# 331658260/Drone-YOLO

Hardware: AMD Instinct MI355X
Metric: images/sec @640x640 Drone-YOLO-s (higher is better)
Workload: dtype fp16; 1 GPU; Drone-YOLO-s (yolov8s-p2-repvgg.yaml, nc=10) inference 640x640: layout+forward+decode+NMS, inputs resident in HBM; fp16 storage / fp32 accumulate (BASELINE config 2 names bf16: bf16 storage fails the IoU >= 0.999 bar - 0.995 - so the headline runs the 16-bit format that meets it; same MFMA rate, same bytes); batch_per_gpu=256, global_batch=256, parallelism=batch-split x1, no collective, hipgraph=True, streams=2, max_det=300

## Files before the change

drone-yolo_amd/csrc/conv3x3_hreg.hip:

```cpp
#include "common_hip.h"
#include "conv_args.h"

namespace DY_NS {


struct HregArgs {
  const void* x;
  const void* w;
  const float* bias;
  const void* res;
  void* y;
  int N, H, W, Cin, ldx, Cout, ldy, ldres, act;
  int tilesX, tilesY, tilesN, nSpatial;
  unsigned x_bytes, y_bytes, r_bytes;
  double* stats;
  const float* bnb_mean;
  const float* bnb_rstd;
  const float* bnb_gamma;
  const float* bnb_beta;
  int bnb_act;
  int dbg;
};

#ifdef DYOLO_ABLATE
#define HR_DBG(bit) (p.dbg & (bit))
#else
#define HR_DBG(bit) 0
#endif

constexpr int kHrTH = 8, kHrTW = 16, kHrHH = 10, kHrHW = 24;
constexpr int kHrStage = 16 * 1024;
constexpr int kHrStages = 3;

template <typename T, int NCH, bool RES, bool STATS = false, bool BNB = false, int BW = 3>
__global__ __launch_bounds__(256, NCH <= 2 ? (BNB ? BW : 3) : 2) void conv3x3_hreg_kernel(const HregArgs p) {
  static_assert(!(BNB && (RES || STATS)), "BNB: its own mode");
  constexpr bool SLOTS = STATS || BNB, RLOAD = RES || BNB;
  constexpr int EPC = Elem<T>::EPC;
  __shared__ __attribute__((aligned(1024))) unsigned char smem[kHrStages * kHrStage];
  __shared__ f32x4 bnc[BNB ? 64 : 1];
  const int tid = threadIdx.x, lane = tid & 63, wave = tid >> 6;
  const int lq = lane >> 4, lr = lane & 15;
  const __amdgpu_buffer_rsrc_t yrs = __builtin_amdgcn_make_buffer_rsrc(p.y, 0, p.y_bytes, 0x00020000);
  const __amdgpu_buffer_rsrc_t rrs = __builtin_amdgcn_make_buffer_rsrc(const_cast<void*>(p.res ? p.res : p.y), 0, p.res ? p.r_bytes : 0u, 0x00020000);

  const int G = (int)gridDim.x;
  const int logical = ((int)blockIdx.x & 7) * (G >> 3) + ((int)blockIdx.x >> 3);
  const int nt = logical % p.tilesN;
  const int sb = logical / p.tilesN, Gs = G / p.tilesN;
  const int myTiles = sb < p.nSpatial ? (p.nSpatial - sb + Gs - 1) / Gs : 0;
  if constexpr (SLOTS) {
    if (blockIdx.x == 0)
      for (int i = tid; i < 2 * p.Cout; i += 256) p.stats[i] = 0.0;
    if (myTiles <= 0 && tid < 128) {
      const int co = nt * 64 + (tid & 63);
      if (co < p.Cout) p.stats[(size_t)(1 + sb) * 2 * p.Cout + (tid >> 6) * p.Cout + co] = 0.0;
    }
  }
  if (myTiles <= 0) return;
  const int nItems = myTiles * NCH;

  u32x4 wreg[NCH][9];
  {
    const u32x4* wg = reinterpret_cast<const u32x4*>(p.w) + (size_t)nt * NCH * 9 * 4 * 64;
#pragma unroll
    for (int c = 0; c < NCH; ++c)
#pragma unroll
      for (int t = 0; t < 9; ++t) wreg[c][t] = wg[((c * 9 + t) * 4 + wave) * 64 + lane];
  }
  const f32x4 bias4 = *reinterpret_cast<const f32x4*>(p.bias + nt * 64 + wave * 16 + lq * 4);

  constexpr int NDMA = 4;
  constexpr unsigned kOob = 0xfffffff0u;
  const unsigned pre = (unsigned)((p.W + 1) * p.ldx) * 2u;
  const __amdgpu_buffer_rsrc_t xrs = __builtin_amdgcn_make_buffer_rsrc(const_cast<char*>(reinterpret_cast<const char*>(p.x)) - pre, 0, p.x_bytes + pre, 0x00020000);
  unsigned rel[NDMA];
  int hyx[NDMA];
#pragma unroll
  for (int k = 0; k < NDMA; ++k) {
    const int s = (k * 4 + wave) * 64 + lane;
    const int pix = s >> 2, part = s & 3;
    const int hy = pix / kHrHW, hx = pix - hy * kHrHW;
    const bool dead = hx >= kHrTW + 2 || hy >= kHrHH;
    rel[k] = dead ? kOob : (unsigned)((hy * p.W + hx) * p.ldx + (part ^ ((hx >> 1) & 3)) * EPC) * 2u;
    hyx[k] = hy | (hx << 8);
  }
  unsigned voff[NDMA];
  unsigned l_base = 0;
  int l_tile = sb, l_chunk = 0, l_item = 0;
  auto setup_tile = [&](int tile) {
    const int tx = tile % p.tilesX;
    const int r = tile / p.tilesX;
    const int ty = r % p.tilesY, n = r / p.tilesY;
    const int y0 = ty * kHrTH, x0 = tx * kHrTW;
    l_base = (unsigned)(((n * p.H + y0) * p.W + x0) * p.ldx) * 2u;
    const bool interior = y0 > 0 && y0 + kHrTH + 1 <= p.H && x0 > 0 && x0 + kHrTW + 1 <= p.W;
    if (interior) {
#pragma unroll
      for (int k = 0; k < NDMA; ++k) voff[k] = rel[k];
    } else {
#pragma unroll
      for (int k = 0; k < NDMA; ++k) {
        const int gy = y0 - 1 + (hyx[k] & 255), gx = x0 - 1 + (hyx[k] >> 8);
        voff[k] = ((unsigned)gy < (unsigned)p.H && (unsigned)gx < (unsigned)p.W) ? rel[k] : kOob;
      }
    }
  };
  auto issue_dma = [&](int stage) {
    unsigned char* sa = smem + stage * kHrStage;
    const bool live = l_item < nItems && !(HR_DBG(4) && l_item >= 2);
    if (live) {
      const unsigned soff = l_base + (unsigned)l_chunk * (4u * EPC * (unsigned)sizeof(T));
#pragma unroll
      for (int k = 0; k < NDMA; ++k)
        __builtin_amdgcn_raw_ptr_buffer_load_lds(xrs, (__attribute__((address_space(3))) void*)(sa + (k * 4 + wave) * 1024), 16, (int)voff[k], (int)soff, 0, 0);
      ++l_item;
      if (++l_chunk == NCH) {
        l_chunk = 0;
        l_tile += Gs;
        if (l_item < nItems) setup_tile(l_tile);
      }
    } else {
#pragma unroll
      for (int k = 0; k < NDMA; ++k)
        __builtin_amdgcn_raw_ptr_buffer_load_lds(xrs, (__attribute__((address_space(3))) void*)(sa + (k * 4 + wave) * 1024), 16, (int)kOob, 0, 0, 0);
    }
  };

  int lane_base[3];
#pragma unroll
  for (int q = 0; q < 3; ++q) lane_base[q] = (lr + q) * 64 + ((lq ^ (((lr + q) >> 1) & 3)) * 16);

  f32x4 acc[kHrTH];
#pragma unroll
  for (int o = 0; o < kHrTH; ++o) acc[o] = bias4;

  auto compute = [&](int stg, int c) {
    const unsigned char* sa = smem + stg * kHrStage;
#pragma unroll
    for (int iy = 0; iy < kHrHH; ++iy) {
      u32x4 a[3];
#pragma unroll
      for (int q = 0; q < 3; ++q) a[q] = *reinterpret_cast<const u32x4*>(sa + lane_base[q] + (HR_DBG(8) ? 0 : iy * (kHrHW * 64)));
#pragma unroll
      for (int r = 0; r < 3; ++r) {
        const int o = iy - r;
        if (o >= 0 && o < kHrTH) {
#pragma unroll
          for (int q = 0; q < 3; ++q) {
            if (HR_DBG(2)) asm volatile("" ::"v"(a[q]));
            else acc[o] = Elem<T>::mma(wreg[c][r * 3 + q], a[q], acc[o]);
          }
        }
      }
    }
  };

  typedef __attribute__((ext_vector_type(4))) T t4;
  u32x4 rl[kHrTH / 2];
  auto load_residual = [&](int tile) {
    const int tx = tile % p.tilesX;
    const int r = tile / p.tilesX;
    const int ty = r % p.tilesY, n = r / p.tilesY;
    const int xx = tx * kHrTW + lr;
    const int co16 = nt * 64 + wave * 16 + (lq >> 1) * 8;
#pragma unroll
    for (int o = 0; o < kHrTH; o += 2) {
      const int yy = ty * kHrTH + o + (lq & 1);
      const bool ok = yy < p.H && xx < p.W;
      const unsigned off = ok ? (unsigned)((((size_t)(n * p.H + yy) * p.W + xx) * (size_t)p.ldres + co16) * sizeof(T)) : 0xfffffff0u;
      rl[o / 2] = __builtin_amdgcn_raw_buffer_load_b128(rrs, off, 0, 0);
    }
  };
  unsigned lane_out[kHrTH / 2];
  {
    const int co16 = nt * 64 + wave * 16 + (lq >> 1) * 8;
#pragma unroll
    for (int o = 0; o < kHrTH; o += 2) lane_out[o / 2] = (unsigned)(((o + (lq & 1)) * p.W + lr) * p.ldy + co16) * (unsigned)sizeof(T);
  }
  float st_sum[4] = {0.f, 0.f, 0.f, 0.f}, st_sq[4] = {0.f, 0.f, 0.f, 0.f};
  if constexpr (BNB) {
    if (tid < 64) {
      const int co = nt * 64 + tid;
      const float mu = p.bnb_mean[co], rs = p.bnb_rstd[co], gr = p.bnb_gamma[co] * rs;
      bnc[tid] = f32x4{rs, -mu * rs, gr, p.bnb_beta[co] - gr * mu};
    }
    asm volatile("s_waitcnt lgkmcnt(0)" ::: "memory");
  }
  auto epilogue = [&](int tile) {
    const int tx = tile % p.tilesX;
    const int r = tile / p.tilesX;
    const int ty = r % p.tilesY, n = r / p.tilesY;
    const int y0 = ty * kHrTH, x0 = tx * kHrTW;
    const unsigned out_base = (unsigned)(((n * p.H + y0) * p.W + x0) * p.ldy) * (unsigned)sizeof(T);
    const bool whole = y0 + kHrTH <= p.H && x0 + kHrTW <= p.W;
    u32x2 pk[kHrTH];
#pragma unroll
    for (int o = 0; o < kHrTH; ++o) {
      float v[4] = {acc[o][0], acc[o][1], acc[o][2], acc[o][3]};
      if (p.act == DY_ACT_SILU) {
#pragma unroll
        for (int e = 0; e < 4; ++e) v[e] = silu_f32(v[e]);
      }
      if constexpr (RES) {
        const auto sx = __builtin_amdgcn_permlane16_swap(rl[o / 2][0], rl[o / 2][2], false, false);
        const auto sy = __builtin_amdgcn_permlane16_swap(rl[o / 2][1], rl[o / 2][3], false, false);
        const t4 rr = __builtin_bit_cast(t4, u32x2{sx[o & 1], sy[o & 1]});
#pragma unroll
        for (int e = 0; e < 4; ++e) v[e] += Elem<T>::to_f32(rr[e]);
      }
      t4 ov;
#pragma unroll
      for (int e = 0; e < 4; ++e) ov[e] = Elem<T>::from_f32(v[e]);
      if constexpr (STATS) {
        if (whole || (y0 + o < p.H && x0 + lr < p.W)) {
#pragma unroll
          for (int e = 0; e < 4; ++e) {
            const float f = Elem<T>::to_f32(ov[e]);
            st_sum[e] += f, st_sq[e] += f * f;
          }
        }
      }
      if constexpr (BNB) {
        const auto sx = __builtin_amdgcn_permlane16_swap(rl[o / 2][0], rl[o / 2][2], false, false);
        const auto sy = __builtin_amdgcn_permlane16_swap(rl[o / 2][1], rl[o / 2][3], false, false);
        const t4 zz = __builtin_bit_cast(t4, u32x2{sx[o & 1], sy[o & 1]});
        if (whole || (y0 + o < p.H && x0 + lr < p.W)) {
#pragma unroll
          for (int e = 0; e < 4; ++e) {
            const f32x4 k = bnc[wave * 16 + lq * 4 + e];
            const float zf = Elem<T>::to_f32(zz[e]);
            const float xh = zf * k[0] + k[1];
            float du = Elem<T>::to_f32(ov[e]);
            if (p.bnb_act == DY_ACT_SILU) {
              const float u = zf * k[2] + k[3];
              const float sg = __builtin_amdgcn_rcpf(1.0f + __builtin_amdgcn_exp2f(u * -1.4426950408889634f));
              du *= sg * (1.0f + u * (1.0f - sg));
            }
            st_sum[e] += du, st_sq[e] += du * xh;
          }
        }
      }
      pk[o] = __builtin_bit_cast(u32x2, ov);
      acc[o] = bias4;
    }
#pragma unroll
    for (int o = 0; o < kHrTH; o += 2) {
      const auto sx = __builtin_amdgcn_permlane16_swap(pk[o][0], pk[o + 1][0], false, false);
      const auto sy = __builtin_amdgcn_permlane16_swap(pk[o][1], pk[o + 1][1], false, false);
      unsigned off = lane_out[o / 2];
      if (!whole) off = (y0 + o + (lq & 1) < p.H && x0 + lr < p.W) ? off : kOob;
      __builtin_amdgcn_raw_buffer_store_b128(u32x4{sx[0], sy[0], sx[1], sy[1]}, yrs, HR_DBG(1) ? kOob : off, (int)out_base, 0);
    }
  };

  setup_tile(l_tile);
  issue_dma(0);
  issue_dma(1 % kHrStages);
  asm volatile("s_waitcnt vmcnt(0)" ::: "memory");
  __builtin_amdgcn_s_barrier();
  int c_tile = sb;
  int stage = 0;
  for (int it = 0; it < nItems; it += NCH) {
#pragma unroll
    for (int c = 0; c < NCH; ++c) {
      if constexpr (RLOAD) {
        if (c == NCH - 1) load_residual(c_tile);
      }
      issue_dma(stage + 2 >= kHrStages ? stage + 2 - kHrStages : stage + 2);
      compute(stage, c);
      if (c == NCH - 1) {
        epilogue(c_tile);
        c_tile += Gs;
      }
      asm volatile("s_waitcnt vmcnt(0)" ::: "memory");
      __builtin_amdgcn_s_barrier();
      stage = stage + 1 == kHrStages ? 0 : stage + 1;
    }
  }
  if constexpr (SLOTS) {
#pragma unroll
    for (int e = 0; e < 4; ++e) {
      float a = st_sum[e], b = st_sq[e];
#pragma unroll
      for (int m = 1; m < 16; m <<= 1) a += __shfl_xor(a, m, 64), b += __shfl_xor(b, m, 64);
      const int co = nt * 64 + wave * 16 + lq * 4 + e;
      if (lr == 0 && co < p.Cout) {
        double* slot = p.stats + (size_t)(1 + sb) * 2 * p.Cout;
        slot[co] = (double)a, slot[p.Cout + co] = (double)b;
      }
    }
  }
}

constexpr int kH2TH = 4, kH2TW = 16, kH2HH = 9, kH2Pitch = 40, kH2PlaneB = 24;
constexpr int kH2Stage = 24 * 1024;

template <typename T, int NCH, bool STATS = false>
__global__ __launch_bounds__(256, 2) void conv3x3_hreg_s2_kernel(const HregArgs p) {
  constexpr int EPC = Elem<T>::EPC;
  __shared__ __attribute__((aligned(1024))) unsigned char smem[kHrStages * kH2Stage];
  const int tid = threadIdx.x, lane = tid & 63, wave = tid >> 6;
  const int lq = lane >> 4, lr = lane & 15;
  const __amdgpu_buffer_rsrc_t yrs = __builtin_amdgcn_make_buffer_rsrc(p.y, 0, p.y_bytes, 0x00020000);
  const int Ho = (p.H - 1) / 2 + 1, Wo = (p.W - 1) / 2 + 1;

  const int G = (int)gridDim.x;
  const int logical = ((int)blockIdx.x & 7) * (G >> 3) + ((int)blockIdx.x >> 3);
  const int nt = logical % p.tilesN;
  const int sb = logical / p.tilesN, Gs = G / p.tilesN;
  const int myTiles = sb < p.nSpatial ? (p.nSpatial - sb + Gs - 1) / Gs : 0;
  if constexpr (STATS) {
    if (blockIdx.x == 0)
      for (int i = tid; i < 2 * p.Cout; i += 256) p.stats[i] = 0.0;
    if (myTiles <= 0 && tid < 128) {
      const int co = nt * 64 + (tid & 63);
      if (co < p.Cout) p.stats[(size_t)(1 + sb) * 2 * p.Cout + (tid >> 6) * p.Cout + co] = 0.0;
    }
  }
  if (myTiles <= 0) return;
  const int nItems = myTiles * NCH;

  u32x4 wreg[NCH][9];
  {
    const u32x4* wg = reinterpret_cast<const u32x4*>(p.w) + (size_t)nt * NCH * 9 * 4 * 64;
#pragma unroll
    for (int c = 0; c < NCH; ++c)
#pragma unroll
      for (int t = 0; t < 9; ++t) wreg[c][t] = wg[((c * 9 + t) * 4 + wave) * 64 + lane];
  }
  const f32x4 bias4 = *reinterpret_cast<const f32x4*>(p.bias + nt * 64 + wave * 16 + lq * 4);

  constexpr int NDMA = 6;
  constexpr unsigned kOob = 0xfffffff0u;
  const unsigned pre = (unsigned)((p.W + 1) * p.ldx) * 2u;
  const __amdgpu_buffer_rsrc_t xrs = __builtin_amdgcn_make_buffer_rsrc(const_cast<char*>(reinterpret_cast<const char*>(p.x)) - pre, 0, p.x_bytes + pre, 0x00020000);
  unsigned rel[NDMA];
  int hyx[NDMA];
#pragma unroll
  for (int k = 0; k < NDMA; ++k) {
    const int s = (k * 4 + wave) * 64 + lane;
    const int slot = s >> 2, part = s & 3;
    const int hy = slot / kH2Pitch, c = slot - hy * kH2Pitch;
    const bool planeB = c >= kH2PlaneB;
    const int ci = planeB ? c - kH2PlaneB : c;
    const int hx = planeB ? 2 * ci + 1 : 2 * ci;
    const bool dead = hy >= kH2HH || hx > 2 * kH2TW;
    rel[k] = dead ? kOob : (unsigned)((hy * p.W + hx) * p.ldx + (part ^ ((ci >> 1) & 3)) * EPC) * 2u;
    hyx[k] = hy | (hx << 8);
  }
  unsigned voff[NDMA];
  unsigned l_base = 0;
  int l_tile = sb, l_chunk = 0, l_item = 0;
  auto setup_tile = [&](int tile) {
    const int tx = tile % p.tilesX;
    const int r = tile / p.tilesX;
    const int ty = r % p.tilesY, n = r / p.tilesY;
    const int y0 = 2 * ty * kH2TH, x0 = 2 * tx * kH2TW;
    l_base = (unsigned)(((n * p.H + y0) * p.W + x0) * p.ldx) * 2u;
    const bool interior = y0 > 0 && y0 - 1 + kH2HH <= p.H && x0 > 0 && x0 + 2 * kH2TW <= p.W;
    if (interior) {
#pragma unroll
      for (int k = 0; k < NDMA; ++k) voff[k] = rel[k];
    } else {
#pragma unroll
      for (int k = 0; k < NDMA; ++k) {
        const int gy = y0 - 1 + (hyx[k] & 255), gx = x0 - 1 + (hyx[k] >> 8);
        voff[k] = ((unsigned)gy < (unsigned)p.H && (unsigned)gx < (unsigned)p.W) ? rel[k] : kOob;
      }
    }
  };
  auto issue_dma = [&](int stage) {
    unsigned char* sa = smem + stage * kH2Stage;
    const bool live = l_item < nItems;
    if (live) {
      const unsigned soff = l_base + (unsigned)l_chunk * (4u * EPC * (unsigned)sizeof(T));
#pragma unroll
      for (int k = 0; k < NDMA; ++k)
        __builtin_amdgcn_raw_ptr_buffer_load_lds(xrs, (__attribute__((address_space(3))) void*)(sa + (k * 4 + wave) * 1024), 16, (int)voff[k], (int)soff, 0, 0);
      ++l_item;
      if (++l_chunk == NCH) {
        l_chunk = 0;
        l_tile += Gs;
        if (l_item < nItems) setup_tile(l_tile);
      }
    } else {
#pragma unroll
      for (int k = 0; k < NDMA; ++k)
        __builtin_amdgcn_raw_ptr_buffer_load_lds(xrs, (__attribute__((address_space(3))) void*)(sa + (k * 4 + wave) * 1024), 16, (int)kOob, 0, 0, 0);
    }
  };

  int lane_base[3];
  lane_base[0] = lr * 64 + ((lq ^ ((lr >> 1) & 3)) * 16);
  lane_base[1] = (kH2PlaneB + lr) * 64 + ((lq ^ ((lr >> 1) & 3)) * 16);
  lane_base[2] = (lr + 1) * 64 + ((lq ^ (((lr + 1) >> 1) & 3)) * 16);

  f32x4 acc[kH2TH];
#pragma unroll
  for (int o = 0; o < kH2TH; ++o) acc[o] = bias4;

  auto compute = [&](int stg, int c) {
    const unsigned char* sa = smem + stg * kH2Stage;
#pragma unroll
    for (int iy = 0; iy < kH2HH; ++iy) {
      u32x4 a[3];
#pragma unroll
      for (int q = 0; q < 3; ++q) a[q] = *reinterpret_cast<const u32x4*>(sa + lane_base[q] + iy * (kH2Pitch * 64));
#pragma unroll
      for (int r = 0; r < 3; ++r) {
        if ((iy - r) % 2 == 0) {
          const int o = (iy - r) / 2;
          if (iy - r >= 0 && o < kH2TH) {
#pragma unroll
            for (int q = 0; q < 3; ++q) acc[o] = Elem<T>::mma(wreg[c][r * 3 + q], a[q], acc[o]);
          }
        }
      }
    }
  };

  typedef __attribute__((ext_vector_type(4))) T t4;
  unsigned lane_out[kH2TH / 2];
  {
    const int co16 = nt * 64 + wave * 16 + (lq >> 1) * 8;
#pragma unroll
    for (int o = 0; o < kH2TH; o += 2) lane_out[o / 2] = (unsigned)(((o + (lq & 1)) * Wo + lr) * p.ldy + co16) * (unsigned)sizeof(T);
  }
  float st_sum[4] = {0.f, 0.f, 0.f, 0.f}, st_sq[4] = {0.f, 0.f, 0.f, 0.f};
  auto epilogue = [&](int tile) {
    const int tx = tile % p.tilesX;
    const int r = tile / p.tilesX;
    const int ty = r % p.tilesY, n = r / p.tilesY;
    const int y0 = ty * kH2TH, x0 = tx * kH2TW;
    const unsigned out_base = (unsigned)(((n * Ho + y0) * Wo + x0) * p.ldy) * (unsigned)sizeof(T);
    const bool whole = y0 + kH2TH <= Ho && x0 + kH2TW <= Wo;
    u32x2 pk[kH2TH];
#pragma unroll
    for (int o = 0; o < kH2TH; ++o) {
      float v[4] = {acc[o][0], acc[o][1], acc[o][2], acc[o][3]};
      if (p.act == DY_ACT_SILU) {
#pragma unroll
        for (int e = 0; e < 4; ++e) v[e] = silu_f32(v[e]);
      }
      t4 ov;
#pragma unroll
      for (int e = 0; e < 4; ++e) ov[e] = Elem<T>::from_f32(v[e]);
      pk[o] = __builtin_bit_cast(u32x2, ov);
      if constexpr (STATS) {
        if (whole || (y0 + o < Ho && x0 + lr < Wo)) {
#pragma unroll
          for (int e = 0; e < 4; ++e) {
            const float f = Elem<T>::to_f32(ov[e]);
            st_sum[e] += f, st_sq[e] += f * f;
          }
        }
      }
      acc[o] = bias4;
    }
#pragma unroll
    for (int o = 0; o < kH2TH; o += 2) {
      const auto sx = __builtin_amdgcn_permlane16_swap(pk[o][0], pk[o + 1][0], false, false);
      const auto sy = __builtin_amdgcn_permlane16_swap(pk[o][1], pk[o + 1][1], false, false);
      unsigned off = lane_out[o / 2];
      if (!whole) off = (y0 + o + (lq & 1) < Ho && x0 + lr < Wo) ? off : kOob;
      __builtin_amdgcn_raw_buffer_store_b128(u32x4{sx[0], sy[0], sx[1], sy[1]}, yrs, off, (int)out_base, 0);
    }
  };

  setup_tile(l_tile);
  issue_dma(0);
  issue_dma(1);
  asm volatile("s_waitcnt vmcnt(0)" ::: "memory");
  __builtin_amdgcn_s_barrier();
  int c_tile = sb;
  int stage = 0;
  for (int it = 0; it < nItems; it += NCH) {
#pragma unroll
    for (int c = 0; c < NCH; ++c) {
      issue_dma(stage + 2 >= kHrStages ? stage + 2 - kHrStages : stage + 2);
      compute(stage, c);
      if (c == NCH - 1) {
        epilogue(c_tile);
        c_tile += Gs;
      }
      asm volatile("s_waitcnt vmcnt(0)" ::: "memory");
      __builtin_amdgcn_s_barrier();
      stage = stage + 1 == kHrStages ? 0 : stage + 1;
    }
  }
  if constexpr (STATS) {
#pragma unroll
    for (int e = 0; e < 4; ++e) {
      float a = st_sum[e], b = st_sq[e];
#pragma unroll
      for (int m = 1; m < 16; m <<= 1) a += __shfl_xor(a, m, 64), b += __shfl_xor(b, m, 64);
      const int co = nt * 64 + wave * 16 + lq * 4 + e;
      if (lr == 0 && co < p.Cout) {
        double* slot = p.stats + (size_t)(1 + sb) * 2 * p.Cout;
        slot[co] = (double)a, slot[p.Cout + co] = (double)b;
      }
    }
  }
}

[[maybe_unused]] constexpr int kBnbWgs = 2;
template <typename T>
static int launch_hreg(const HregArgs& a, hipStream_t st) {
  HregArgs p = a;
  const int nch = p.Cin / 32;
  int grid = 256 * (nch <= 2 ? 3 : 2);
  const long long nwork = (long long)p.nSpatial * p.tilesN;
  if (nwork < grid) grid = (int)nwork;
  const int q = 8 * p.tilesN;
  grid = (grid + q - 1) / q * q;
  const bool res = p.res != nullptr;
#ifndef DYOLO_L2E_BUILD
  if (p.bnb_mean) {
    static const int bw = dy_ablate("DYOLO_BNB_WGS") ? dy_ablate("DYOLO_BNB_WGS") : kBnbWgs;
    if (nch == 2 && bw == 2) {
      int g2 = 256 * 2;
      if (nwork < g2) g2 = (int)nwork;
      grid = (g2 + q - 1) / q * q;
      hipLaunchKernelGGL((conv3x3_hreg_kernel<T, 2, false, false, true, 2>), dim3((unsigned)grid), dim3(256), 0, st, p);
    } else if (nch == 2) {
      hipLaunchKernelGGL((conv3x3_hreg_kernel<T, 2, false, false, true, 3>), dim3((unsigned)grid), dim3(256), 0, st, p);
    } else {
      hipLaunchKernelGGL((conv3x3_hreg_kernel<T, 4, false, false, true>), dim3((unsigned)grid), dim3(256), 0, st, p);
    }
    note_stats(grid / p.tilesN);
    return check_launch("conv3x3_hreg_kernel<bnb>");
  }
#endif
  if (p.stats) {
    if (nch == 1) hipLaunchKernelGGL((conv3x3_hreg_kernel<T, 1, false, true>), dim3((unsigned)grid), dim3(256), 0, st, p);
    else if (nch == 2) hipLaunchKernelGGL((conv3x3_hreg_kernel<T, 2, false, true>), dim3((unsigned)grid), dim3(256), 0, st, p);
    else hipLaunchKernelGGL((conv3x3_hreg_kernel<T, 4, false, true>), dim3((unsigned)grid), dim3(256), 0, st, p);
    note_stats(grid / p.tilesN);
    return check_launch("conv3x3_hreg_kernel");
  }
  if (nch == 1) {
    if (res) hipLaunchKernelGGL((conv3x3_hreg_kernel<T, 1, true>), dim3((unsigned)grid), dim3(256), 0, st, p);
    else hipLaunchKernelGGL((conv3x3_hreg_kernel<T, 1, false>), dim3((unsigned)grid), dim3(256), 0, st, p);
  } else if (nch == 2) {
    if (res) hipLaunchKernelGGL((conv3x3_hreg_kernel<T, 2, true>), dim3((unsigned)grid), dim3(256), 0, st, p);
    else hipLaunchKernelGGL((conv3x3_hreg_kernel<T, 2, false>), dim3((unsigned)grid), dim3(256), 0, st, p);
  } else {
    hipLaunchKernelGGL((conv3x3_hreg_kernel<T, 4, false>), dim3((unsigned)grid), dim3(256), 0, st, p);
  }
  return check_launch("conv3x3_hreg_kernel");
}

template <typename T>
static int launch_hreg_s2(const HregArgs& a, hipStream_t st) {
  HregArgs p = a;
  int grid = 256 * 2;
  const long long nwork = (long long)p.nSpatial * p.tilesN;
  if (nwork < grid) grid = (int)nwork;
  const int q = 8 * p.tilesN;
  grid = (grid + q - 1) / q * q;
#ifndef DYOLO_L2E_BUILD
  if (p.stats) {
    hipLaunchKernelGGL((conv3x3_hreg_s2_kernel<T, 2, true>), dim3((unsigned)grid), dim3(256), 0, st, p);
    note_stats(grid / p.tilesN);
    return check_launch("conv3x3_hreg_s2_kernel");
  }
#endif
  hipLaunchKernelGGL((conv3x3_hreg_s2_kernel<T, 2>), dim3((unsigned)grid), dim3(256), 0, st, p);
  return check_launch("conv3x3_hreg_s2_kernel");
}

int conv3x3_hreg_try(const dy_conv_desc* d, hipStream_t st) {
  static const int off = dy_ablate("DYOLO_NO_HREG");
  if (off) return 1;
  if (!(d->dtype == DY_BF16 || d->dtype == DY_F16) || d->out_f32 || d->ksize != 3 || d->pad != 1 || d->groups > 1 || d->up2x || d->x2) return 1;
  if (d->stride == 2) {
    if (d->cin != 64 || d->cout % 64 != 0 || d->cout > 256 || d->residual) return 1;
    const long long xb2 = (long long)d->batch * d->h * d->w_in * d->ld_x * 2, yb2 = (long long)d->batch * d->ho * d->wo * d->ld_y * 2;
    if (xb2 >= (1ll << 31) || yb2 >= (1ll << 32) - 64 || d->ld_y % 8 || (reinterpret_cast<uintptr_t>(d->y) & 15)) return 1;
    HregArgs a{};
    a.x = d->x, a.w = d->w, a.bias = d->bias, a.res = nullptr, a.y = d->y;
    a.N = d->batch, a.H = d->h, a.W = d->w_in, a.Cin = d->cin, a.ldx = d->ld_x, a.Cout = d->cout, a.ldy = d->ld_y, a.ldres = 0, a.act = d->act;
    a.tilesX = (d->wo + kH2TW - 1) / kH2TW;
    a.tilesY = (d->ho + kH2TH - 1) / kH2TH;
    a.tilesN = d->cout / 64;
    a.nSpatial = d->batch * a.tilesY * a.tilesX;
    a.x_bytes = (unsigned)xb2, a.y_bytes = (unsigned)yb2, a.r_bytes = 0;
    a.stats = (d->y_dtype1 || d->bnb_z) ? nullptr : d->bn_stats;
    return d->dtype == DY_BF16 ? launch_hreg_s2<bf16_t>(a, st) : launch_hreg_s2<f16_t>(a, st);
  }
  if (d->stride != 1) return 1;
  if ((d->cin != 64 && d->cin != 128) || d->cout % 64 != 0 || d->cout > 256 || d->residual) return 1;
  if (d->ho != d->h || d->wo != d->w_in) return 1;
  const long long xb = (long long)d->batch * d->h * d->w_in * d->ld_x * 2, yb = (long long)d->batch * d->ho * d->wo * d->ld_y * 2;
  const long long rb = d->residual ? (long long)d->batch * d->ho * d->wo * d->ld_res * 2 : 0;
  if (xb >= (1ll << 31) || yb >= (1ll << 32) - 64 || rb >= (1ll << 32) - 64) return 1;
  if (d->ld_y % 8 || (reinterpret_cast<uintptr_t>(d->y) & 15) || (d->residual && (d->ld_res % 8 || (reinterpret_cast<uintptr_t>(d->residual) & 15)))) return 1;
  HregArgs a{};
  a.x = d->x, a.w = d->w, a.bias = d->bias, a.res = d->residual, a.y = d->y;
  a.N = d->batch, a.H = d->h, a.W = d->w_in, a.Cin = d->cin, a.ldx = d->ld_x, a.Cout = d->cout, a.ldy = d->ld_y, a.ldres = d->ld_res, a.act = d->act;
  a.tilesX = (d->wo + kHrTW - 1) / kHrTW;
  a.tilesY = (d->ho + kHrTH - 1) / kHrTH;
  a.tilesN = d->cout / 64;
  a.nSpatial = d->batch * a.tilesY * a.tilesX;
  a.x_bytes = (unsigned)xb, a.y_bytes = (unsigned)yb, a.r_bytes = (unsigned)rb;
  a.stats = d->bn_stats;
  if (d->bnb_z) {
    const long long zb = (long long)d->batch * d->ho * d->wo * d->bnb_ld_z * 2;
#ifdef DYOLO_L2E_BUILD
    const bool built = false;
#else
    const bool built = d->bn_stats && !d->y_dtype1 && d->act == DY_ACT_NONE && d->cin != 32 && zb < (1ll << 32) - 64 && d->bnb_ld_z % 8 == 0 && (reinterpret_cast<uintptr_t>(d->bnb_z) & 15) == 0;
#endif
    if (built) {
      a.res = d->bnb_z, a.ldres = d->bnb_ld_z, a.r_bytes = (unsigned)zb;
      a.bnb_mean = d->bnb_mean, a.bnb_rstd = d->bnb_rstd, a.bnb_gamma = d->bnb_gamma, a.bnb_beta = d->bnb_beta, a.bnb_act = d->bnb_act;
    } else {
      a.stats = nullptr;
    }
  }
  a.dbg = dy_ablate("DYOLO_DBG");
  return d->dtype == DY_BF16 ? launch_hreg<bf16_t>(a, st) : launch_hreg<f16_t>(a, st);
}

}
```

Baseline: 21110 images/sec.

## Compute 128 output channels per staged input tile in register-weight 3x3 conv

Adds two wider output-channel groupings to the register-resident-weight 3x3 conv. For Cin=64 the kernel holds two 64-channel weight fragments per wave and issues two MMAs per staged activation fragment. For Cin=128 it runs 8 waves per workgroup, each half covering a different 64-channel group. Either way one LDS-staged input tile serves 128 output channels, which halves the input re-fetch and staging traffic for layers without residual or stats. The cost is higher register pressure or lower occupancy, plus extra bias handling through LDS.

```diff
diff --git a/drone-yolo_amd/csrc/conv3x3_hreg.hip b/drone-yolo_amd/csrc/conv3x3_hreg.hip
--- a/drone-yolo_amd/csrc/conv3x3_hreg.hip
+++ b/drone-yolo_amd/csrc/conv3x3_hreg.hip
@@ -32,14 +32,19 @@
 constexpr int kHrStage = 16 * 1024;
 constexpr int kHrStages = 3;
 
-template <typename T, int NCH, bool RES, bool STATS = false, bool BNB = false, int BW = 3>
-__global__ __launch_bounds__(256, NCH <= 2 ? (BNB ? BW : 3) : 2) void conv3x3_hreg_kernel(const HregArgs p) {
+template <typename T, int NCH, bool RES, bool STATS = false, bool BNB = false, int BW = 3, int NF = 1, int NW = 4>
+__global__ __launch_bounds__(64 * NW, NW == 8 ? 1 : NF == 2 ? 2 : NCH <= 2 ? (BNB ? BW : 3) : 2) void conv3x3_hreg_kernel(const HregArgs p) {
   static_assert(!(BNB && (RES || STATS)), "BNB: its own mode");
+  static_assert((NF == 1 && NW == 4) || !(RES || STATS || BNB), "the 128-cout groupings: inference without a residual");
+  static_assert((NF == 1 || NF == 2) && (NW == 4 || NW == 8) && !(NF == 2 && NW == 8), "one grouping at a time");
   constexpr bool SLOTS = STATS || BNB, RLOAD = RES || BNB;
   constexpr int EPC = Elem<T>::EPC;
+  constexpr int GH = NF * (NW / 4);
   __shared__ __attribute__((aligned(1024))) unsigned char smem[kHrStages * kHrStage];
   __shared__ f32x4 bnc[BNB ? 64 : 1];
+  __shared__ f32x4 biasl[NF == 2 ? 32 : 1];
   const int tid = threadIdx.x, lane = tid & 63, wave = tid >> 6;
+  const int frag = NW == 8 ? wave & 3 : wave;
   const int lq = lane >> 4, lr = lane & 15;
   const __amdgpu_buffer_rsrc_t yrs = __builtin_amdgcn_make_buffer_rsrc(p.y, 0, p.y_bytes, 0x00020000);
   const __amdgpu_buffer_rsrc_t rrs = __builtin_amdgcn_make_buffer_rsrc(const_cast<void*>(p.res ? p.res : p.y), 0, p.res ? p.r_bytes : 0u, 0x00020000);
@@ -60,17 +65,24 @@
   if (myTiles <= 0) return;
   const int nItems = myTiles * NCH;
 
-  u32x4 wreg[NCH][9];
-  {
-    const u32x4* wg = reinterpret_cast<const u32x4*>(p.w) + (size_t)nt * NCH * 9 * 4 * 64;
+  const int g64 = nt * GH + (NW == 8 ? wave >> 2 : 0);
+  u32x4 wreg[NF][NCH][9];
+  f32x4 bias4[NF];
+#pragma unroll
+  for (int f = 0; f < NF; ++f) {
+    const u32x4* wg = reinterpret_cast<const u32x4*>(p.w) + (size_t)(g64 + f) * NCH * 9 * 4 * 64;
 #pragma unroll
     for (int c = 0; c < NCH; ++c)
 #pragma unroll
-      for (int t = 0; t < 9; ++t) wreg[c][t] = wg[((c * 9 + t) * 4 + wave) * 64 + lane];
-  }
-  const f32x4 bias4 = *reinterpret_cast<const f32x4*>(p.bias + nt * 64 + wave * 16 + lq * 4);
-
-  constexpr int NDMA = 4;
+      for (int t = 0; t < 9; ++t) wreg[f][c][t] = wg[((c * 9 + t) * 4 + frag) * 64 + lane];
+    if constexpr (NF == 1) bias4[f] = *reinterpret_cast<const f32x4*>(p.bias + (g64 + f) * 64 + frag * 16 + lq * 4);
+  }
+  if constexpr (NF == 2) {
+    if (tid < 128) reinterpret_cast<float*>(biasl)[tid] = p.bias[nt * 128 + tid];
+    asm volatile("s_waitcnt lgkmcnt(0)" ::: "memory");
+  }
+
+  constexpr int NDMA = 16 / NW;
   constexpr unsigned kOob = 0xfffffff0u;
   const unsigned pre = (unsigned)((p.W + 1) * p.ldx) * 2u;
   const __amdgpu_buffer_rsrc_t xrs = __builtin_amdgcn_make_buffer_rsrc(const_cast<char*>(reinterpret_cast<const char*>(p.x)) - pre, 0, p.x_bytes + pre, 0x00020000);
@@ -78,7 +90,7 @@
   int hyx[NDMA];
 #pragma unroll
   for (int k = 0; k < NDMA; ++k) {
-    const int s = (k * 4 + wave) * 64 + lane;
+    const int s = (k * NW + wave) * 64 + lane;
     const int pix = s >> 2, part = s & 3;
     const int hy = pix / kHrHW, hx = pix - hy * kHrHW;
     const bool dead = hx >= kHrTW + 2 || hy >= kHrHH;
@@ -101,7 +113,14 @@
     } else {
 #pragma unroll
       for (int k = 0; k < NDMA; ++k) {
-        const int gy = y0 - 1 + (hyx[k] & 255), gx = x0 - 1 + (hyx[k] >> 8);
+        int hy = hyx[k] & 255, hx = hyx[k] >> 8;
+        if constexpr (NF == 2) {
+          int t = tid;
+          asm volatile("" : "+v"(t));
+          const int pix = k * NW * 16 + (t >> 2);
+          hy = pix / kHrHW, hx = pix - hy * kHrHW;
+        }
+        const int gy = y0 - 1 + hy, gx = x0 - 1 + hx;
         voff[k] = ((unsigned)gy < (unsigned)p.H && (unsigned)gx < (unsigned)p.W) ? rel[k] : kOob;
       }
     }
@@ -113,7 +132,7 @@
       const unsigned soff = l_base + (unsigned)l_chunk * (4u * EPC * (unsigned)sizeof(T));
 #pragma unroll
       for (int k = 0; k < NDMA; ++k)
-        __builtin_amdgcn_raw_ptr_buffer_load_lds(xrs, (__attribute__((address_space(3))) void*)(sa + (k * 4 + wave) * 1024), 16, (int)voff[k], (int)soff, 0, 0);
+        __builtin_amdgcn_raw_ptr_buffer_load_lds(xrs, (__attribute__((address_space(3))) void*)(sa + (k * NW + wave) * 1024), 16, (int)voff[k], (int)soff, 0, 0);
       ++l_item;
       if (++l_chunk == NCH) {
         l_chunk = 0;
@@ -123,7 +142,7 @@
     } else {
 #pragma unroll
       for (int k = 0; k < NDMA; ++k)
-        __builtin_amdgcn_raw_ptr_buffer_load_lds(xrs, (__attribute__((address_space(3))) void*)(sa + (k * 4 + wave) * 1024), 16, (int)kOob, 0, 0, 0);
+        __builtin_amdgcn_raw_ptr_buffer_load_lds(xrs, (__attribute__((address_space(3))) void*)(sa + (k * NW + wave) * 1024), 16, (int)kOob, 0, 0, 0);
     }
   };
 
@@ -131,12 +150,20 @@
 #pragma unroll
   for (int q = 0; q < 3; ++q) lane_base[q] = (lr + q) * 64 + ((lq ^ (((lr + q) >> 1) & 3)) * 16);
 
-  f32x4 acc[kHrTH];
-#pragma unroll
-  for (int o = 0; o < kHrTH; ++o) acc[o] = bias4;
+  f32x4 acc[NF][kHrTH] = {};
+  if constexpr (NF == 1) {
+#pragma unroll
+    for (int o = 0; o < kHrTH; ++o) acc[0][o] = bias4[0];
+  }
 
   auto compute = [&](int stg, int c) {
     const unsigned char* sa = smem + stg * kHrStage;
+    if constexpr (NF == 2) {
+      if (c == 0) {
+#pragma unroll
+        for (int f = 0; f < NF; ++f) bias4[f] = biasl[f * 16 + frag * 4 + lq];
+      }
+    }
 #pragma unroll
     for (int iy = 0; iy < kHrHH; ++iy) {
       u32x4 a[3];
@@ -149,7 +176,11 @@
 #pragma unroll
           for (int q = 0; q < 3; ++q) {
             if (HR_DBG(2)) asm volatile("" ::"v"(a[q]));
-            else acc[o] = Elem<T>::mma(wreg[c][r * 3 + q], a[q], acc[o]);
+            else {
+              const bool first = NF == 2 && c == 0 && r == 0 && q == 0;
+#pragma unroll
+              for (int f = 0; f < NF; ++f) acc[f][o] = Elem<T>::mma(wreg[f][c][r * 3 + q], a[q], first ? bias4[f] : acc[f][o]);
+            }
           }
         }
       }
@@ -163,7 +194,7 @@
     const int r = tile / p.tilesX;
     const int ty = r % p.tilesY, n = r / p.tilesY;
     const int xx = tx * kHrTW + lr;
-    const int co16 = nt * 64 + wave * 16 + (lq >> 1) * 8;
+    const int co16 = g64 * 64 + frag * 16 + (lq >> 1) * 8;
 #pragma unroll
     for (int o = 0; o < kHrTH; o += 2) {
       const int yy = ty * kHrTH + o + (lq & 1);
@@ -174,7 +205,7 @@
   };
   unsigned lane_out[kHrTH / 2];
   {
-    const int co16 = nt * 64 + wave * 16 + (lq >> 1) * 8;
+    const int co16 = g64 * 64 + frag * 16 + (lq >> 1) * 8;
 #pragma unroll
     for (int o = 0; o < kHrTH; o += 2) lane_out[o / 2] = (unsigned)(((o + (lq & 1)) * p.W + lr) * p.ldy + co16) * (unsigned)sizeof(T);
   }
@@ -194,10 +225,11 @@
     const int y0 = ty * kHrTH, x0 = tx * kHrTW;
     const unsigned out_base = (unsigned)(((n * p.H + y0) * p.W + x0) * p.ldy) * (unsigned)sizeof(T);
     const bool whole = y0 + kHrTH <= p.H && x0 + kHrTW <= p.W;
-    u32x2 pk[kHrTH];
-#pragma unroll
-    for (int o = 0; o < kHrTH; ++o) {
-      float v[4] = {acc[o][0], acc[o][1], acc[o][2], acc[o][3]};
+    u32x2 pk[NF][kHrTH];
+#pragma unroll
+    for (int fo = 0; fo < NF * kHrTH; ++fo) {
+      const int f = fo / kHrTH, o = fo % kHrTH;
+      float v[4] = {acc[f][o][0], acc[f][o][1], acc[f][o][2], acc[f][o][3]};
       if (p.act == DY_ACT_SILU) {
 #pragma unroll
         for (int e = 0; e < 4; ++e) v[e] = silu_f32(v[e]);
@@ -241,16 +273,17 @@
           }
         }
       }
-      pk[o] = __builtin_bit_cast(u32x2, ov);
-      acc[o] = bias4;
-    }
-#pragma unroll
-    for (int o = 0; o < kHrTH; o += 2) {
-      const auto sx = __builtin_amdgcn_permlane16_swap(pk[o][0], pk[o + 1][0], false, false);
-      const auto sy = __builtin_amdgcn_permlane16_swap(pk[o][1], pk[o + 1][1], false, false);
-      unsigned off = lane_out[o / 2];
+      pk[f][o] = __builtin_bit_cast(u32x2, ov);
+      if constexpr (NF == 1) acc[f][o] = bias4[f];
+    }
+#pragma unroll
+    for (int fo = 0; fo < NF * kHrTH; fo += 2) {
+      const int f = fo / kHrTH, o = fo % kHrTH;
+      const auto sx = __builtin_amdgcn_permlane16_swap(pk[f][o][0], pk[f][o + 1][0], false, false);
+      const auto sy = __builtin_amdgcn_permlane16_swap(pk[f][o][1], pk[f][o + 1][1], false, false);
+      unsigned off = lane_out[NF == 2 ? 0 : o / 2] + (unsigned)(f * 64 * (int)sizeof(T));
       if (!whole) off = (y0 + o + (lq & 1) < p.H && x0 + lr < p.W) ? off : kOob;
-      __builtin_amdgcn_raw_buffer_store_b128(u32x4{sx[0], sy[0], sx[1], sy[1]}, yrs, HR_DBG(1) ? kOob : off, (int)out_base, 0);
+      __builtin_amdgcn_raw_buffer_store_b128(u32x4{sx[0], sy[0], sx[1], sy[1]}, yrs, HR_DBG(1) ? kOob : off, (int)(out_base + (NF == 2 ? (unsigned)(o * p.W * p.ldy) * (unsigned)sizeof(T) : 0u)), 0);
     }
   };
 
@@ -515,6 +548,24 @@
   const int q = 8 * p.tilesN;
   grid = (grid + q - 1) / q * q;
   const bool res = p.res != nullptr;
+  if (!res && !p.stats && !p.bnb_mean && p.Cout % 128 == 0 && nch >= 2) {
+    static const int force = dy_ablate("DYOLO_HREG_FORM");
+    const bool wide = force ? force == 2 : nch == 2;
+    if (wide) {
+      p.tilesN = p.Cout / 128;
+      const int q2 = 8 * p.tilesN;
+      int g = nch == 2 ? 512 : 256;
+      const long long nw2 = (long long)p.nSpatial * p.tilesN;
+      if (nw2 < g) g = (int)nw2;
+      g = (g + q2 - 1) / q2 * q2;
+      if (nch == 2) {
+        hipLaunchKernelGGL((conv3x3_hreg_kernel<T, 2, false, false, false, 3, 2, 4>), dim3((unsigned)g), dim3(256), 0, st, p);
+        return check_launch("conv3x3_hreg_kernel<nf2>");
+      }
+      hipLaunchKernelGGL((conv3x3_hreg_kernel<T, 4, false, false, false, 3, 1, 8>), dim3((unsigned)g), dim3(512), 0, st, p);
+      return check_launch("conv3x3_hreg_kernel<w8>");
+    }
+  }
 #ifndef DYOLO_L2E_BUILD
   if (p.bnb_mean) {
     static const int bw = dy_ablate("DYOLO_BNB_WGS") ? dy_ablate("DYOLO_BNB_WGS") : kBnbWgs;
```

New measurement: 21130 images/sec (median of 6 runs). No clear change (+0.1%).
